# mfkiwl/msckf_stereo_c

Hardware: AMD Instinct MI355X
Metric: stereo frames/sec/node on EuRoC-shape input; ATE RMSE vs CPU ref (higher is better)
Workload: dtype f64

## Files before the change

### msckf_stereo_c_amd/csrc/hip/ekf_linalg.hip

```cpp
#include <mutex>
#include <type_traits>
#include "ekf_device.h"
#include "ekf_cap.h"
#include "chol_block.h"

typedef double v4f64 __attribute__((ext_vector_type(4)));

#define QR_BIAS_LIMIT 1e-6
__device__ __forceinline__ bool ekf_direct_wanted(const EkfStreamDev &S) { return ekf_mode_direct(S.qr_mode, S.rows_out[0], S.rows_out[2]); }
__device__ __forceinline__ bool ekf_skip_gram(const EkfStreamDev &S) { return ekf_mode_householder(S.qr_mode) || ekf_direct_wanted(S); }
__device__ __forceinline__ bool ekf_direct(const EkfStreamDev &S) { return (S.rows_out[3] & 4) != 0; }

template <int MODE> struct GemmTraits;
template <> struct GemmTraits<GM_GRAM> { static constexpr bool TA = true,  SYM = true,  KMIN_I = false, KMIN_J = false; };
template <> struct GemmTraits<GM_T>    { static constexpr bool TA = true,  SYM = false, KMIN_I = true,  KMIN_J = false; };
template <> struct GemmTraits<GM_S2>   { static constexpr bool TA = false, SYM = true,  KMIN_I = false, KMIN_J = true;  };
template <> struct GemmTraits<GM_PUPD> { static constexpr bool TA = true,  SYM = true,  KMIN_I = false, KMIN_J = false; };

#define GT 32
#ifndef GK
#define GK 32
#endif
#define GNE (GK / 8)

template <int MODE>
__global__ __launch_bounds__(256) void k_ekf_gemm(const EkfStreamDev *streams) {
    using TR = GemmTraits<MODE>;
    const EkfStreamDev &S = streams[blockIdx.y];
    if (S.n_feat <= 0) return;
    if (MODE != GM_PUPD && (S.route & EKF_ROUTE_SMALL)) return;
    const int d = S.d, ld = S.ld;
    int gram_tile_i = 0, gram_tile_j = 0;
    EkfCapResult cap = {0, 0, 0, 0ULL};
    if (MODE == GM_GRAM) {
        int tg = 1;
        while ((tg + 1) * (tg + 1) <= (int)gridDim.x) ++tg;
        gram_tile_i = (int)blockIdx.x / tg; gram_tile_j = (int)blockIdx.x - gram_tile_i * tg;
        if (gram_tile_j > gram_tile_i || gram_tile_i * GT > S.na_max) return;
        cap = ekf_cap_local(S, blockIdx.x == 0);
        if (ekf_mode_householder(S.qr_mode) || ekf_mode_direct(S.qr_mode, cap.stacked, cap.na)) return;
    }
    const int na = MODE == GM_GRAM ? cap.na : S.rows_out[2];
    const int *__restrict__ act = S.act;
    const double *__restrict__ A; const double *__restrict__ B; double *C;
    int M, N, K;
    double alpha = 1.0, beta = 0.0, diag_add = 0.0;
    if (MODE == GM_GRAM)      { A = S.Hs; B = S.Hs; C = S.S; M = N = na + 1; K = cap.end; }
    const int nk = MODE == GM_GRAM ? 0 : S.rows_out[4];
    const bool direct = MODE != GM_GRAM && MODE != GM_PUPD && ekf_direct(S);
    if (MODE == GM_T)         { A = direct ? S.Hs : S.S;  B = S.P;  C = S.T; M = nk; N = d; K = na; }
    else if (MODE == GM_S2)   { A = S.T;  B = direct ? S.Hs : S.S;  C = S.W; M = N = nk; K = na; diag_add = S.sigma2; }
    else if (MODE == GM_PUPD) { A = S.T;  B = S.T;  C = S.P; M = N = d; K = nk; alpha = -1.0; beta = 1.0; }
    const int tiles_n = (N + GT - 1) / GT, tiles_m = (M + GT - 1) / GT;
    const int tile = blockIdx.x;
    if (MODE == GM_PUPD && tile >= tiles_m * tiles_n) {
        const int c0 = (tile - tiles_m * tiles_n) * GT;
        if (c0 >= d) return;
        const double *Y = S.T;
        __shared__ double s_part[8][GT + 1];
        const int cl = threadIdx.x & 31, ks = threadIdx.x >> 5;
        const int c = c0 + cl;
        double s2 = 0;
        if (c < d)
            for (int k = ks; k < nk; k += 8) s2 += Y[(size_t)k * ld + c] * Y[(size_t)k * ld + d];
        s_part[ks][cl] = s2;
        __syncthreads();
        if (ks == 0 && c < d) {
            double t = 0;
#pragma unroll
            for (int q = 0; q < 8; ++q) t += s_part[q][cl];
            S.delta_x[c] = t;
        }
        return;
    }
    if (MODE != GM_GRAM && tile >= tiles_m * tiles_n) return;
    const int ti = MODE == GM_GRAM ? gram_tile_i : tile / tiles_n, tj = MODE == GM_GRAM ? gram_tile_j : tile - ti * tiles_n;
    if (MODE == GM_GRAM && ti >= tiles_m) return;
    if (TR::SYM && tj > ti) return;
    const int i0 = ti * GT, j0 = tj * GT;
    __shared__ double sA[GK][GT + 1];
    __shared__ double sB[GK][GT + 1];
    const int tid = threadIdx.x, lane = tid & 63, wave = tid >> 6;
    const int wi = (wave >> 1) * 16, wj = (wave & 1) * 16;
    const int lo = tid & 31, hi = tid >> 5;
    int k_begin = 0;
    if (TR::KMIN_I && !direct) k_begin = (i0 / GK) * GK;
    if (TR::KMIN_J && !direct) k_begin = (j0 / GK) * GK;
    const int k_end = K;
    int colA = i0 + lo, colB = j0 + lo;
    if (MODE == GM_GRAM) {
        colA = (i0 + lo < na) ? ekf_act_column(cap.clones, i0 + lo) : d;
        colB = (j0 + lo < na) ? ekf_act_column(cap.clones, j0 + lo) : d;
    }
    const int cloneA = MODE == GM_GRAM ? (colA < d ? (colA - EKF_IMU_DIM) / 6 : -1) : 0;
    const int cloneB = MODE == GM_GRAM ? (colB < d ? (colB - EKF_IMU_DIM) / 6 : -1) : 0;
    const unsigned long long *__restrict__ rowmask = S.rowmask;
    const int *__restrict__ rowidx = S.act + S.ld;
    double ra[GNE], rb[GNE];
    auto fetch = [&](int k0) {
#pragma unroll
        for (int e = 0; e < GNE; ++e) {
            if (MODE == GM_GRAM) {
                const int gk = k0 + hi + 8 * e;
                double v = 0.0, w = 0.0;
                if (gk < K) {
                    const unsigned long long rm = rowmask[gk];
                    const bool onA = cloneA < 0 ? rm != 0ULL : ((rm >> cloneA) & 1ULL) != 0ULL;
                    const bool onB = cloneB < 0 ? rm != 0ULL : ((rm >> cloneB) & 1ULL) != 0ULL;
                    if (onA && i0 + lo < M) v = A[(size_t)gk * ld + colA];
                    if (onB && j0 + lo < N) w = B[(size_t)gk * ld + colB];
                }
                ra[e] = v; rb[e] = w;
                continue;
            }
            const int ii = TR::TA ? lo : hi + 8 * (e / (GK / 32)), kk = TR::TA ? hi + 8 * e : lo + 32 * (e % (GK / 32));
            const int gi = i0 + ii, gk = k0 + kk;
            double v = 0.0;
            if (gi < M && gk < K && !(TR::KMIN_I && !direct && gk < gi)) {
                if (MODE == GM_S2) v = A[(size_t)gi * ld + act[gk]];
                else if (MODE == GM_T && direct) {
                    const int col = act[gk], ri = rowidx[gi];
                    if ((rowmask[ri] >> ((col - EKF_IMU_DIM) / 6)) & 1ULL) v = A[(size_t)ri * ld + col];
                }
                else v = A[(size_t)gk * ld + (MODE == GM_GRAM ? colA : gi)];
            }
            ra[e] = v;
            const int gj = j0 + lo, gkb = k0 + hi + 8 * e;
            double w = 0.0;
            if (gj < N && gkb < K && !(TR::KMIN_J && !direct && gkb < gj)) {
                if (MODE == GM_T) w = B[(size_t)act[gkb] * ld + gj];
                else if (MODE == GM_S2 && direct) {
                    const int col = act[gkb], rj = rowidx[gj];
                    if ((rowmask[rj] >> ((col - EKF_IMU_DIM) / 6)) & 1ULL) w = B[(size_t)rj * ld + col];
                }
                else w = B[(size_t)gkb * ld + (MODE == GM_GRAM ? colB : gj)];
            }
            rb[e] = w;
        }
    };
    v4f64 acc = {0.0, 0.0, 0.0, 0.0};
    if (k_begin < k_end) fetch(k_begin);
    for (int k0 = k_begin; k0 < k_end; k0 += GK) {
        __syncthreads();
#pragma unroll
        for (int e = 0; e < GNE; ++e) {
            if (TR::TA) sA[hi + 8 * e][lo] = ra[e]; else sA[lo + 32 * (e % (GK / 32))][hi + 8 * (e / (GK / 32))] = ra[e];
            sB[hi + 8 * e][lo] = rb[e];
        }
        __syncthreads();
        if (k0 + GK < k_end) fetch(k0 + GK);
#pragma unroll
        for (int s = 0; s < GK / 4; ++s) {
            const int kk = 4 * s + (lane >> 4);
            const double a = sA[kk][wi + (lane & 15)];
            const double b = sB[kk][wj + (lane & 15)];
            acc = __builtin_amdgcn_mfma_f64_16x16x4f64(a, b, acc, 0, 0, 0);
        }
    }
#pragma unroll
    for (int r = 0; r < 4; ++r) {
        const int i = i0 + wi + (lane >> 4) + 4 * r;
        const int j = j0 + wj + (lane & 15);
        if (i >= M || j >= N) continue;
        if (TR::SYM && j > i) continue;
        double v = alpha * acc[r];
        if (MODE == GM_PUPD) v += beta * C[(size_t)i * ld + j];
        if (i == j) v += diag_add;
        C[(size_t)i * ld + j] = v;
        if (TR::SYM && i != j) C[(size_t)j * ld + i] = v;
        if (MODE == GM_PUPD && i == j && i >= 12 && i < 15 && S.pos_var_out) S.pos_var_out[i - 12] = v;
    }
}

template <int Q> __device__ __forceinline__ double qr_lane_sum(double v) {
    auto bfly = [](double x, auto ctrl) {
        const long long b = __double_as_longlong(x);
        const int lo = __builtin_amdgcn_update_dpp(0, (int)b, decltype(ctrl)::value, 0xf, 0xf, true);
        const int hi = __builtin_amdgcn_update_dpp(0, (int)(b >> 32), decltype(ctrl)::value, 0xf, 0xf, true);
        return x + __longlong_as_double(((long long)hi << 32) | (unsigned int)lo);
    };
    v = bfly(v, std::integral_constant<int, 0xB1>());
    v = bfly(v, std::integral_constant<int, 0x4E>());
    if (Q == 8) v = bfly(v, std::integral_constant<int, 0x141>());
    return v;
}
template <int Q, int RL, class ColOf, class RAt>
__device__ __forceinline__ void tsqr_wide(const EkfStreamDev &S, int n1, int K, ColOf colOf, RAt Rat, double *sB) {
    constexpr int BR = Q * RL;
    const int tid = threadIdx.x, nth = blockDim.x, ld = S.ld;
    const int q = tid & (Q - 1), g = tid / Q, ng = nth / Q;
    for (int k0 = 0; k0 < K; k0 += BR) {
        __syncthreads();
        for (int e = tid; e < BR * n1; e += nth) {
            const int r = e / n1, c = e - r * n1, gk = k0 + r;
            double v = 0.0;
            if (gk < K) {
                int col, clone;
                colOf(c, col, clone);
                const unsigned long long rm = S.rowmask[gk];
                const bool on = clone < 0 ? rm != 0ULL : ((rm >> clone) & 1ULL) != 0ULL;
                if (on) v = S.Hs[(size_t)gk * ld + col];
            }
            sB[e] = v;
        }
        __syncthreads();
        double *own = sB + (size_t)q * RL * n1;
        for (int k = 0; k < n1; ++k) {
            double bk[RL];
            double ss = 0.0;
#pragma unroll
            for (int i = 0; i < RL; ++i) { bk[i] = own[i * n1 + k]; ss += bk[i] * bk[i]; }
            ss = qr_lane_sum<Q>(ss);
            const double x0 = Rat(k, k);
            if (ss < 1e-200 || ss < 1e-40 * (x0 * x0)) continue;
            const double nrm = sqrt(x0 * x0 + ss);
            const double alpha = x0 > 0.0 ? -nrm : nrm;
            const double v0 = x0 - alpha;
            const double beta = 2.0 / (v0 * v0 + ss);
            for (int j = k + 1 + g; j < n1; j += ng) {
                double bj[RL];
                double dot = 0.0;
#pragma unroll
                for (int i = 0; i < RL; ++i) { bj[i] = own[i * n1 + j]; dot += bk[i] * bj[i]; }
                const double rkj = Rat(k, j);
                const double t = beta * (qr_lane_sum<Q>(dot) + v0 * rkj);
#pragma unroll
                for (int i = 0; i < RL; ++i) own[i * n1 + j] = bj[i] - t * bk[i];
                if (q == 0) Rat(k, j) = rkj - t * v0;
            }
            __syncthreads();
            if (tid == 0) Rat(k, k) = alpha;
        }
    }
    __syncthreads();
}
template <class ColOf, class RAt>
__device__ __forceinline__ void tsqr_quads(const EkfStreamDev &S, int n1, int K, ColOf colOf, RAt Rat, double *sB, int room) {
    if (room >= 48 * n1) tsqr_wide<4, 12>(S, n1, K, colOf, Rat, sB);
    else if (room >= 32 * n1) tsqr_wide<4, 8>(S, n1, K, colOf, Rat, sB);
    else tsqr_wide<4, 4>(S, n1, K, colOf, Rat, sB);
}

__device__ __forceinline__ int ekf_compress_entry(const EkfStreamDev &S, int *s_w ) {
    const int na = S.rows_out[2], me = S.rows_out[1], d = S.d, ld = S.ld;
    if (na <= 0) { if (threadIdx.x == 0) S.rows_out[3] = 0; return 1; }
    if (ekf_direct_wanted(S)) {
        int *rowidx = S.act + ld;
        const int tid = threadIdx.x, lane = tid & 63, wave = tid >> 6, nw = (int)blockDim.x >> 6;
        int base = 0;
        for (int r0 = 0; r0 < me; r0 += (int)blockDim.x) {
            const int r = r0 + tid;
            const bool on = r < me && S.rowmask[r] != 0ULL;
            const unsigned long long b = __ballot(on);
            if (lane == 0) s_w[wave] = __popcll(b);
            __syncthreads();
            int off = base, tot = 0;
            for (int w = 0; w < nw; ++w) { const int c = s_w[w]; if (w < wave) off += c; tot += c; }
            if (on && off + __popcll(b & ((1ULL << lane) - 1ULL)) < ld) rowidx[off + __popcll(b & ((1ULL << lane) - 1ULL))] = r;
            base += tot;
            __syncthreads();
        }
        __threadfence_block();
        __syncthreads();
        for (int i = tid; i < base; i += (int)blockDim.x) S.T[(size_t)i * ld + d] = S.Hs[(size_t)rowidx[i] * ld + d];
        if (tid == 0) { S.rows_out[3] = 4; S.rows_out[4] = base; }
        return 1;
    }
    return ekf_skip_gram(S) ? 2 : 0;
}
template <class RAt>
__device__ __forceinline__ void ekf_compress_exit(const EkfStreamDev &S, bool gram_done, int diag, RAt Rat, double *sB, int room) {
    const int na = S.rows_out[2], n1 = na + 1, K = S.rows_out[1], d = S.d, ld = S.ld;
    const int tid = threadIdx.x, nth = blockDim.x;
    const bool need = ekf_mode_householder(S.qr_mode) || (S.qr_mode == 0 && (!gram_done || (diag & 2)));
    if (!need) { if (tid == 0) S.rows_out[3] = diag; return; }
    __syncthreads();
    for (int e = tid; e < n1 * n1; e += nth) { const int k = e / n1, j = e - k * n1; if (j >= k) Rat(k, j) = 0.0; }
    const int *act = S.act;
    tsqr_quads(S, n1, K, [=](int c, int &col, int &clone) { col = c < na ? act[c] : d; clone = c < na ? (col - EKF_IMU_DIM) / 6 : -1; }, Rat, sB, room);
    for (int e = tid; e < na * na; e += nth) {
        const int i = e / na, j = e - i * na;
        if (j <= i) S.S[(size_t)i * ld + j] = Rat(j, i);
    }
    for (int k = tid; k < na; k += nth) S.T[(size_t)k * ld + d] = Rat(k, na);
    if (tid == 0) S.rows_out[3] = diag | 1;
}

#define TQ_THREADS 512
__device__ __forceinline__ double tq_rows_sum(double v) {
    {
        const unsigned long long b = (unsigned long long)__double_as_longlong(v);
        const auto lo = __builtin_amdgcn_permlane16_swap((unsigned)b, (unsigned)b, false, false), hi = __builtin_amdgcn_permlane16_swap((unsigned)(b >> 32), (unsigned)(b >> 32), false, false);
        v = __longlong_as_double((long long)(((unsigned long long)hi[0] << 32) | lo[0])) + __longlong_as_double((long long)(((unsigned long long)hi[1] << 32) | lo[1]));
    }
    {
        const unsigned long long b = (unsigned long long)__double_as_longlong(v);
        const auto lo = __builtin_amdgcn_permlane32_swap((unsigned)b, (unsigned)b, false, false), hi = __builtin_amdgcn_permlane32_swap((unsigned)(b >> 32), (unsigned)(b >> 32), false, false);
        v = __longlong_as_double((long long)(((unsigned long long)hi[0] << 32) | lo[0])) + __longlong_as_double((long long)(((unsigned long long)hi[1] << 32) | lo[1]));
    }
    return v;
}
__device__ __forceinline__ double tq_rcp(double x) {
    double r = __builtin_amdgcn_rcp(x);
    r = __builtin_fma(__builtin_fma(-x, r, 1.0), r, r);
    r = __builtin_fma(__builtin_fma(-x, r, 1.0), r, r);
    return r;
}
template <int C, bool FIRST> __device__ __forceinline__ void tq_fmac_bcast(double &acc, double x, double a) {
    if (FIRST) asm("s_nop 4\n\tv_fmac_f64_dpp %0, %1, %2 row_newbcast:%3 row_mask:0xf bank_mask:0xf" : "+v"(acc) : "v"(x), "v"(a), "n"(C));
    else asm("v_fmac_f64_dpp %0, %1, %2 row_newbcast:%3 row_mask:0xf bank_mask:0xf" : "+v"(acc) : "v"(x), "v"(a), "n"(C));
}
template <int RL, int I = 0> struct TqDot {
    static __device__ __forceinline__ void run(double (&p)[4], const double (&vr)[RL / 16], const double (&bc)[RL]) {
        tq_fmac_bcast<I % 16, I == 0>(p[I & 3], vr[I / 16], bc[I]);
        TqDot<RL, I + 1>::run(p, vr, bc);
    }
};
template <int RL> struct TqDot<RL, RL> { static __device__ __forceinline__ void run(double (&)[4], const double (&)[RL / 16], const double (&)[RL]) {} };
template <int RL, int I = 0> struct TqAxpy {
    static __device__ __forceinline__ void run(double (&bc)[RL], const double (&vr)[RL / 16], double ntt) {
        tq_fmac_bcast<I % 16, I == 0>(bc[I], vr[I / 16], ntt);
        TqAxpy<RL, I + 1>::run(bc, vr, ntt);
    }
};
template <int RL> struct TqAxpy<RL, RL> { static __device__ __forceinline__ void run(double (&)[RL], const double (&)[RL / 16], double) {} };
template <int RL>
__device__ __forceinline__ void tq_form_reflector(const double (&bc)[RL], double x0, double *sVs, int *sFlag_s, double *Rkk, int r) {
    double p0 = 0.0, p1 = 0.0, p2 = 0.0, p3 = 0.0;
#pragma unroll
    for (int i = 0; i < RL; i += 4) { p0 = __builtin_fma(bc[i], bc[i], p0); p1 = __builtin_fma(bc[i + 1], bc[i + 1], p1); p2 = __builtin_fma(bc[i + 2], bc[i + 2], p2); p3 = __builtin_fma(bc[i + 3], bc[i + 3], p3); }
    const double ss = tq_rows_sum((p0 + p1) + (p2 + p3));
    const bool skip = ss < 1e-200 || ss < 1e-40 * (x0 * x0);
    if (!skip) {
        const double n2 = __builtin_fma(x0, x0, ss);
        const double nrm = n2 * rsqrt_nr(n2);
        const double alpha = x0 > 0.0 ? -nrm : nrm;
        const double v0 = x0 - alpha;
        const double beta = 2.0 * tq_rcp(__builtin_fma(v0, v0, ss));
#pragma unroll
        for (int i = 0; i < RL; i += 2) *reinterpret_cast<double2 *>(sVs + r * RL + i) = make_double2(bc[i], bc[i + 1]);
        if (r == 0) { sVs[4 * RL] = v0; sVs[4 * RL + 1] = beta; *Rkk = alpha; }
    }
    if (r == 0) *sFlag_s = skip ? 0 : 1;
}
template <int RL, int NC>
__device__ __forceinline__ void tsqr_regs(const EkfStreamDev &S, int na, int K, double *Rg, double *sV, int *sFlag) {
    static_assert(RL % 16 == 0, "a DPP row holds the reflector's entries of its rows, 16 per register");
    constexpr int BR = 4 * RL, NW = TQ_THREADS / 64, SLAB = 16 * NW, VS = BR + 2, VR = RL / 16;
    const int n1 = na + 1, d = S.d, ld = S.ld;
    const int tid = threadIdx.x, lane = tid & 63, r = lane >> 4, c = lane & 15;
    const int wave = __builtin_amdgcn_readfirstlane(tid >> 6);
    int col[NC], clone[NC];
    bool has[NC];
#pragma unroll
    for (int t = 0; t < NC; ++t) {
        const int j = 16 * wave + c + SLAB * t;
        has[t] = j < n1;
        col[t] = j < na ? S.act[j] : d;
        clone[t] = j < na ? (col[t] - EKF_IMU_DIM) / 6 : -1;
    }
    for (int e = tid; e < n1 * n1; e += TQ_THREADS) { const int k = e / n1, j = e - k * n1; if (j >= k) Rg[(size_t)k * ld + j] = 0.0; }
    __syncthreads();
    for (int k0 = 0; k0 < K; k0 += BR) {
        double b[NC][RL];
#pragma unroll
        for (int i = 0; i < RL; ++i) {
            const int gk = k0 + r * RL + i;
            const unsigned long long rm = gk < K ? S.rowmask[gk] : 0ULL;
#pragma unroll
            for (int t = 0; t < NC; ++t) {
                const bool on = has[t] && (clone[t] < 0 ? rm != 0ULL : ((rm >> clone[t]) & 1ULL) != 0ULL);
                b[t][i] = on ? S.Hs[(size_t)gk * ld + col[t]] : 0.0;
            }
        }
        double ra[NC], rb[NC], rc[NC];
#pragma unroll
        for (int t = 0; t < NC; ++t) {
            const int j = 16 * wave + c + SLAB * t;
            ra[t] = has[t] ? Rg[j] : 0.0;
            rb[t] = has[t] && n1 > 1 ? Rg[(size_t)ld + j] : 0.0;
        }
        if (wave == 0 && c == 0) tq_form_reflector<RL>(b[0], ra[0], sV, sFlag, Rg, r);
        __syncthreads();
        for (int k = 0; k < n1; ++k) {
            const int s = k & 1;
            const double *vs = sV + s * VS;
            double vr[VR];
#pragma unroll
            for (int m = 0; m < VR; ++m) vr[m] = vs[r * RL + 16 * m + c];
            const double v0 = vs[BR], beta = vs[BR + 1];
            const bool live = __builtin_amdgcn_readfirstlane(sFlag[s]) != 0;
#pragma unroll
            for (int t = 0; t < NC; ++t) { const int j = 16 * wave + c + SLAB * t; rc[t] = (has[t] && k + 2 < n1) ? Rg[(size_t)(k + 2) * ld + j] : 0.0; }
            auto apply = [&](double (&bc)[RL], double rkj, int j, bool on) {
                double p[4] = {0.0, 0.0, 0.0, 0.0};
                TqDot<RL>::run(p, vr, bc);
                const double dot = tq_rows_sum((p[0] + p[1]) + (p[2] + p[3]));
                const double tt = on ? beta * __builtin_fma(v0, rkj, dot) : 0.0;
                TqAxpy<RL>::run(bc, vr, -tt);
                if (on && r == 0) Rg[(size_t)k * ld + j] = __builtin_fma(-tt, v0, rkj);
            };
            const int k1 = k + 1;
            const int w1 = (k1 & (SLAB - 1)) >> 4, c1 = k1 & 15, t1 = k1 / SLAB;
            const bool own_wave = k1 < n1 && wave == w1;
#pragma unroll
            for (int t = 0; t < NC; ++t) {
                if (own_wave && t1 == t) {
                    const int j = 16 * wave + c + SLAB * t;
                    if (live) apply(b[t], ra[t], j, has[t] && j > k);
                    if (c == c1) tq_form_reflector<RL>(b[t], rb[t], sV + (s ^ 1) * VS, sFlag + (s ^ 1), Rg + (size_t)k1 * ld + k1, r);
                }
            }
            if (live) {
#pragma unroll
                for (int t = 0; t < NC; ++t) {
                    const int j0 = 16 * wave + SLAB * t;
                    if (!(own_wave && t1 == t) && j0 + 15 > k && j0 < n1) apply(b[t], ra[t], j0 + c, has[t] && j0 + c > k);
                }
            }
#pragma unroll
            for (int t = 0; t < NC; ++t) { ra[t] = rb[t]; rb[t] = rc[t]; }
            __syncthreads();
        }
    }
}
template <int RL, int NC, class Load>
__device__ __forceinline__ void tsqr_wave(int n1, int n_blocks, int first, int stride, Load load, double *R, int ldr, double *sVw, int *sFlagw) {
    constexpr int BR = 4 * RL, VR = RL / 16;
    const int lane = threadIdx.x & 63, r = lane >> 4, c = lane & 15;
    for (int blk = first; blk < n_blocks; blk += stride) {
        double b[NC][RL];
#pragma unroll
        for (int i = 0; i < RL; ++i) {
#pragma unroll
            for (int t = 0; t < NC; ++t) b[t][i] = load(blk, r * RL + i, c + 16 * t);
        }
        for (int k = 0; k < n1; ++k) {
            const int tk = k >> 4, ck = k & 15;
#pragma unroll
            for (int t = 0; t < NC; ++t)
                if (tk == t && c == ck) tq_form_reflector<RL>(b[t], R[k * ldr + k], sVw, sFlagw, R + k * ldr + k, r);
            __builtin_amdgcn_wave_barrier();
            double vr[VR];
#pragma unroll
            for (int m = 0; m < VR; ++m) vr[m] = sVw[r * RL + 16 * m + c];
            const double v0 = sVw[BR], beta = sVw[BR + 1];
            const bool live = __builtin_amdgcn_readfirstlane(*sFlagw) != 0;
            if (live) {
#pragma unroll
                for (int t = 0; t < NC; ++t) {
                    if (16 * t + 15 > k && 16 * t < n1) {
                        const int j = c + 16 * t;
                        const bool on = j < n1 && j > k;
                        const double rkj = on ? R[k * ldr + j] : 0.0;
                        double p[4] = {0.0, 0.0, 0.0, 0.0};
                        TqDot<RL>::run(p, vr, b[t]);
                        const double dot = tq_rows_sum((p[0] + p[1]) + (p[2] + p[3]));
                        const double tt = on ? beta * __builtin_fma(v0, rkj, dot) : 0.0;
                        TqAxpy<RL>::run(b[t], vr, -tt);
                        if (on && r == 0) R[k * ldr + j] = __builtin_fma(-tt, v0, rkj);
                    }
                }
            }
            __builtin_amdgcn_wave_barrier();
        }
    }
}
template <int RL, int NC, int WPE>
__global__ __launch_bounds__(TQ_THREADS, WPE) void k_ekf_tsqr(const EkfStreamDev *streams, int do_cap) {
    const EkfStreamDev &S = streams[blockIdx.y];
    if (S.n_feat <= 0 || (S.route & EKF_ROUTE_SMALL)) return;
    if (!ekf_mode_householder(S.qr_mode)) return;
    if (do_cap) { (void)ekf_cap_local<TQ_THREADS>(S, true); __syncthreads(); }
    __shared__ int s_w[TQ_THREADS / 64];
    __shared__ __attribute__((aligned(16))) double sV[2 * (4 * RL + 2)];
    __shared__ int sFlag[2];
    if (ekf_compress_entry(S, s_w) != 2) return;
    const int na = S.rows_out[2], K = S.rows_out[1], d = S.d, ld = S.ld;
    const int tid = threadIdx.x;
    if (na + 1 > (TQ_THREADS / 4) * NC) { if (tid == 0) S.rows_out[3] = 0x80; return; }
    double *Rg = S.W;
    tsqr_regs<RL, NC>(S, na, K, Rg, sV, sFlag);
    for (int e = tid; e < na * na; e += TQ_THREADS) {
        const int i = e / na, j = e - i * na;
        if (j <= i) S.S[(size_t)i * ld + j] = Rg[(size_t)j * ld + i];
    }
    for (int k = tid; k < na; k += TQ_THREADS) S.T[(size_t)k * ld + d] = Rg[(size_t)k * ld + na];
    if (tid == 0) S.rows_out[3] = 1;
}

#define CHOLG_THREADS 512
__global__ __launch_bounds__(CHOLG_THREADS) void k_ekf_chol(const EkfStreamDev *streams, int which, int pan_rs) {
    const EkfStreamDev &S = streams[blockIdx.y];
    if (S.n_feat <= 0 || (S.route & EKF_ROUTE_SMALL)) return;
    int entry = 0;
    __shared__ int s_w[CHOLG_THREADS / 64];
    if (which == 0) {
        if (ekf_mode_householder(S.qr_mode)) return;
        entry = ekf_compress_entry(S, s_w);
        if (entry == 1) return;
    }
    const int n = which == 0 ? S.rows_out[2] : S.rows_out[4];
    const int nt = n + (which == 0 ? 1 : 0);
    const int lda = S.ld;
    double *A = which == 0 ? S.S : S.W;
    extern __shared__ double s_dyn[];
    double *sPanT = s_dyn;
    __shared__ double s_tol, s_mx[CHOLG_THREADS / 64];
    __shared__ int s_diag;
    __shared__ CholBlockShared s_cb;
    const int tid = threadIdx.x;
    if (tid == 0) s_diag = 0;
    for (int e = tid; e < LNB * pan_rs; e += CHOLG_THREADS) sPanT[e] = 0.0;
    if (which == 0) {
        double mx = 0;
        for (int i = tid; i < n; i += CHOLG_THREADS) mx = fmax(mx, A[(size_t)i * lda + i]);
        for (int off = 32; off > 0; off >>= 1) mx = fmax(mx, __shfl_xor(mx, off));
        if ((tid & 63) == 0) s_mx[tid >> 6] = mx;
        __syncthreads();
        if (tid == 0) { double m = 0; for (int i = 0; i < CHOLG_THREADS / 64; ++i) m = fmax(m, s_mx[i]); s_tol = m * (double)S.d * 1e-14; }
        __syncthreads();
        const double lam = s_tol;
        for (int i = tid; i < n; i += CHOLG_THREADS) A[(size_t)i * lda + i] += lam;
    }
    __syncthreads();
    chol_blocked_lds<CHOLG_THREADS / 64>(A, [lda](int i, int j) { return i * lda + j; }, n, nt, 0.0, sPanT, pan_rs, s_cb);
    if (which == 0) {
        int tiny = 0;
        for (int i = tid; i < n; i += CHOLG_THREADS) { const double l = A[(size_t)i * lda + i]; tiny += (l * l < 100.0 * s_tol) ? 1 : 0; }
        for (int o = 32; o > 0; o >>= 1) tiny += __shfl_xor(tiny, o);
        __shared__ int s_tiny[CHOLG_THREADS / 64];
        if ((tid & 63) == 0) s_tiny[tid >> 6] = tiny;
        __syncthreads();
        double pm = 0;
        for (int i = tid; i < n; i += CHOLG_THREADS) pm = fmax(pm, S.P[(size_t)S.act[i] * lda + S.act[i]]);
        for (int o = 32; o > 0; o >>= 1) pm = fmax(pm, __shfl_xor(pm, o));
        __syncthreads();
        if ((tid & 63) == 0) s_mx[tid >> 6] = pm;
        __syncthreads();
        if (tid == 0) {
            int t = 0; for (int i = 0; i < CHOLG_THREADS / 64; ++i) t += s_tiny[i];
            double p = 0; for (int i = 0; i < CHOLG_THREADS / 64; ++i) p = fmax(p, s_mx[i]);
            s_diag = (t << 8) | ((s_tol * p > QR_BIAS_LIMIT * S.sigma2) ? 2 : 0);
        }
        for (int k = tid; k < n; k += CHOLG_THREADS) S.T[(size_t)k * lda + S.d] = A[(size_t)n * lda + k];
        __syncthreads();
        double *Rg = S.W;
        ekf_compress_exit(S, true, s_diag, [=](int k, int j) -> double & { return Rg[(size_t)k * lda + j]; }, sPanT, LNB * pan_rs);
    }
}

#define CHOL_LDS_MAX_ROWS 181
#define CHOL_THREADS 512
#define CHOL_WAVES (CHOL_THREADS / 64)
#define CHOL_PAN_RS 192

__device__ __forceinline__ int pk(int i, int j) { return i * (i + 1) / 2 + j; }

__global__ __launch_bounds__(CHOL_THREADS) void k_ekf_chol_lds(const EkfStreamDev *streams, int which, int lds_doubles) {
    const EkfStreamDev &S = streams[blockIdx.y];
    if (S.n_feat <= 0 || (S.route & EKF_ROUTE_SMALL)) return;
    int entry = 0;
    __shared__ int s_w[CHOL_WAVES];
    if (which == 0) {
        if (ekf_mode_householder(S.qr_mode)) return;
        entry = ekf_compress_entry(S, s_w);
        if (entry == 1) return;
    }
    double *A = which == 0 ? S.S : S.W;
    const int off = 0, lda = S.ld;
    const int n = which == 0 ? S.rows_out[2] : S.rows_out[4];
    const int nt = n + (which == 0 ? 1 : 0);
    const bool semidef = which == 0;
    extern __shared__ double s_dyn[];
    double *sM = s_dyn;
    double *sPanT = s_dyn + nt * (nt + 1) / 2;
    __shared__ double s_tol, s_mx[CHOL_WAVES];
    __shared__ int s_diag;
    __shared__ CholBlockShared s_cb;
    const int tid = threadIdx.x, lane = tid & 63, wave = tid >> 6;
    if (tid == 0) s_diag = 0;
    auto Rl = [=](int k, int j) -> double & { return sM[k * nt - k * (k - 1) / 2 + (j - k)]; };
    const int room = lds_doubles - nt * (nt + 1) / 2;
    for (int i0 = wave * 8; i0 < nt; i0 += CHOL_WAVES * 8) {
        double v[8][3];
#pragma unroll
        for (int u = 0; u < 8; ++u) {
            const int i = i0 + u;
            const double *src = A + (size_t)(off + i) * lda + off;
#pragma unroll
            for (int k = 0; k < 3; ++k) { const int j = lane + 64 * k; v[u][k] = (i < nt && j <= i) ? src[j] : 0.0; }
        }
#pragma unroll
        for (int u = 0; u < 8; ++u) {
            const int i = i0 + u;
            if (i >= nt) continue;
            double *dst = sM + pk(i, 0);
#pragma unroll
            for (int k = 0; k < 3; ++k) { const int j = lane + 64 * k; if (j <= i) dst[j] = v[u][k]; }
        }
    }
    for (int e = tid; e < LNB * CHOL_PAN_RS; e += CHOL_THREADS) sPanT[e] = 0.0;
    __syncthreads();
    if (semidef) {
        double mx = 0;
        for (int i = tid; i < n; i += CHOL_THREADS) mx = fmax(mx, sM[pk(i, i)]);
        for (int o = 32; o > 0; o >>= 1) mx = fmax(mx, __shfl_xor(mx, o));
        if (lane == 0) s_mx[wave] = mx;
        __syncthreads();
        if (tid == 0) { double m = 0; for (int i = 0; i < CHOL_WAVES; ++i) m = fmax(m, s_mx[i]); s_tol = m * (double)S.d * 1e-14; }
        __syncthreads();
        const double lam = s_tol;
        for (int i = tid; i < n; i += CHOL_THREADS) sM[pk(i, i)] += lam;
        __syncthreads();
    }
    const double tol = 0.0;
    chol_blocked_lds<CHOL_WAVES>(sM, [](int i, int j) { return pk(i, j); }, n, nt, tol, sPanT, CHOL_PAN_RS, s_cb);
    if (which == 0) {
        int tiny = 0;
        for (int i = tid; i < n; i += CHOL_THREADS) { const double l = sM[pk(i, i)]; tiny += (l * l < 100.0 * s_tol) ? 1 : 0; }
        for (int o = 32; o > 0; o >>= 1) tiny += __shfl_xor(tiny, o);
        __shared__ int s_tiny[CHOL_WAVES];
        if (lane == 0) s_tiny[wave] = tiny;
        __syncthreads();
        double pm = 0;
        for (int i = tid; i < n; i += CHOL_THREADS) pm = fmax(pm, S.P[(size_t)S.act[i] * lda + S.act[i]]);
        for (int o = 32; o > 0; o >>= 1) pm = fmax(pm, __shfl_xor(pm, o));
        __syncthreads();
        if (lane == 0) s_mx[wave] = pm;
        __syncthreads();
        if (tid == 0) {
            int t = 0; for (int i = 0; i < CHOL_WAVES; ++i) t += s_tiny[i];
            double p = 0; for (int i = 0; i < CHOL_WAVES; ++i) p = fmax(p, s_mx[i]);
            s_diag = (t << 8) | ((s_tol * p > QR_BIAS_LIMIT * S.sigma2) ? 2 : 0);
        }
    }
    for (int i = wave; i < nt; i += CHOL_WAVES) {
        double *dst = A + (size_t)(off + i) * lda + off;
        const double *src = sM + pk(i, 0);
#pragma unroll
        for (int k = 0; k < 3; ++k) { const int j = lane + 64 * k; if (j <= i && j < n) dst[j] = src[j]; }
    }
    if (which == 0) {
        for (int k = tid; k < n; k += CHOL_THREADS) S.T[(size_t)k * lda + S.d] = sM[pk(n, k)];
        __syncthreads();
        ekf_compress_exit(S, true, s_diag, Rl, sPanT, room);
    }
}

#define QR_MAX_N1 (6 * 64 + 1)
#define TS_COLS 32
#define TS_RB 16
__global__ __launch_bounds__(256) void k_ekf_trsm(const EkfStreamDev *streams) {
    const EkfStreamDev &S = streams[blockIdx.y];
    if (S.n_feat <= 0 || (S.route & EKF_ROUTE_SMALL)) return;
    const int n = S.rows_out[4], ld = S.ld, ncols = S.d + 1;
    const int c0 = blockIdx.x * TS_COLS;
    if (c0 >= ncols) return;
    const double *L = S.W;
    double *B = S.T;
    extern __shared__ double s_dyn[];
    double *sL = s_dyn;
    double *sY = s_dyn + (size_t)TS_RB * (n + 1);
    const int tid = threadIdx.x, c = tid & 31, r8 = tid >> 5;
    for (int e = tid; e < n * TS_COLS; e += 256) {
        const int i = e >> 5, cc = e & 31;
        sY[e] = (c0 + cc < ncols) ? B[(size_t)i * ld + c0 + cc] : 0.0;
    }
    constexpr int LPF = 14;
    const int lrow = tid >> 4, lr = tid & 15;
    double lpf[LPF];
    auto fetch_L = [&](int ib) {
        const int nb = min(TS_RB, n - ib), wcols = ib + nb;
#pragma unroll
        for (int q = 0; q < LPF; ++q) {
            const int p = lr + 16 * q;
            lpf[q] = (lrow < nb && p < wcols) ? L[(size_t)(ib + lrow) * ld + p] : 0.0;
        }
    };
    const bool l_fits = n + TS_RB <= 16 * LPF;
    if (l_fits) fetch_L(0);
    for (int ib = 0; ib < n; ib += TS_RB) {
        const int nb = min(TS_RB, n - ib);
        __syncthreads();
        if (l_fits) {
#pragma unroll
            for (int q = 0; q < LPF; ++q) {
                const int p = lr + 16 * q;
                if (lrow < nb && p < ib + nb) sL[(size_t)lrow * (n + 1) + p] = lpf[q];
            }
            if (ib + TS_RB < n) fetch_L(ib + TS_RB);
        } else {
            for (int e = tid; e < nb * (ib + nb); e += 256) {
                const int i = e / (ib + nb), p = e - i * (ib + nb);
                sL[(size_t)i * (n + 1) + p] = L[(size_t)(ib + i) * ld + p];
            }
        }
        __syncthreads();
        double acc0 = 0.0, acc1 = 0.0;
        {
            const double *l0 = sL + (size_t)r8 * (n + 1), *l1 = sL + (size_t)(r8 + 8) * (n + 1);
            for (int p = 0; p < ib; ++p) {
                const double y = sY[p * TS_COLS + c];
                acc0 += l0[p] * y;
                acc1 += l1[p] * y;
            }
        }
        if (r8 < nb) sY[(ib + r8) * TS_COLS + c] -= acc0;
        if (r8 + 8 < nb) sY[(ib + r8 + 8) * TS_COLS + c] -= acc1;
        __syncthreads();
        if (tid < TS_COLS) {
            double x[TS_RB];
#pragma unroll
            for (int j = 0; j < TS_RB; ++j) {
                x[j] = 0.0;
                if (j < nb) {
                    double s2 = sY[(ib + j) * TS_COLS + tid];
                    const double *lj = sL + (size_t)j * (n + 1) + ib;
#pragma unroll
                    for (int cc = 0; cc < j; ++cc) s2 -= lj[cc] * x[cc];
                    x[j] = (lj[j] != 0.0) ? s2 / lj[j] : 0.0;
                    sY[(ib + j) * TS_COLS + tid] = x[j];
                }
            }
        }
    }
    __syncthreads();
    for (int e = tid; e < n * TS_COLS; e += 256) {
        const int i = e >> 5, cc = e & 31;
        if (c0 + cc < ncols) B[(size_t)i * ld + c0 + cc] = sY[e];
    }
}

#define SU_CH 128
__global__ __launch_bounds__(256) void k_ekf_small_update(const EkfStreamDev *streams) {
    const EkfStreamDev &S = streams[blockIdx.y];
    if (S.n_feat <= 0 || !(S.route & EKF_ROUTE_SMALL)) return;
    const EkfCapResult cap = ekf_cap_local(S, true);
    const int d = S.d, ld = S.ld, na = cap.na, n1 = na + 1, K = cap.end;
    const int tid = threadIdx.x;
    if (na <= 0 || na > SU_MAX_NA) {
        for (int c = tid; c < d; c += 256) S.delta_x[c] = 0.0;
        return;
    }
    extern __shared__ double s_dyn[];
    double *sT = s_dyn;
    double *sG = sT + (size_t)na * (d + 1);
    double *sS = sG + n1 * n1;
    double *sC = sS + na * na;
    __shared__ int s_col[SU_MAX_NA + 1], s_clone[SU_MAX_NA + 1];
    __shared__ double s_lam;
    if (tid < n1) {
        const int col = tid < na ? ekf_act_column(cap.clones, tid) : d;
        s_col[tid] = col;
        s_clone[tid] = tid < na ? (col - EKF_IMU_DIM) / 6 : -1;
    }
    __syncthreads();
    const bool hh_only = ekf_mode_householder(S.qr_mode);
    if (tid == 0) s_lam = 0.0;
    if (!hh_only) {
    const int np = n1 * (n1 + 1) / 2;
    const int groups = np <= 128 ? 256 / np : 1;
    int pi[2], pj[2], pg[2];
    double acc[2] = {0.0, 0.0};
    for (int q = 0; q < 2; ++q) {
        int p = tid + 256 * q, grp = 0;
        if (groups > 1) { grp = q == 0 ? tid / np : groups; p = tid - grp * np; }
        pg[q] = (groups > 1) ? (grp < groups ? grp : -1) : (p < np ? 0 : -1);
        if (pg[q] < 0) p = 0;
        int i = 0;
        while ((i + 1) * (i + 2) / 2 <= p) ++i;
        pi[q] = i; pj[q] = p - i * (i + 1) / 2;
    }
    for (int k0 = 0; k0 < K; k0 += SU_CH) {
        __syncthreads();
        for (int e = tid; e < SU_CH * n1; e += 256) {
            const int r = e / n1, c = e - r * n1, gk = k0 + r;
            double v = 0.0;
            if (gk < K) {
                const unsigned long long rm = S.rowmask[gk];
                const bool on = s_clone[c] < 0 ? rm != 0ULL : ((rm >> s_clone[c]) & 1ULL) != 0ULL;
                if (on) v = S.Hs[(size_t)gk * ld + s_col[c]];
            }
            sC[e] = v;
        }
        __syncthreads();
        for (int q = 0; q < 2; ++q) {
            if (pg[q] < 0) continue;
            double a = acc[q];
            for (int r = pg[q]; r < SU_CH; r += groups) a += sC[r * n1 + pi[q]] * sC[r * n1 + pj[q]];
            acc[q] = a;
        }
    }
    __syncthreads();
    if (groups > 1) {
        if (pg[0] >= 0) sC[pg[0] * np + (pi[0] * (pi[0] + 1) / 2 + pj[0])] = acc[0];
        __syncthreads();
        if (pg[0] == 0) {
            const int p = pi[0] * (pi[0] + 1) / 2 + pj[0];
            double t = 0.0;
            for (int g2 = 0; g2 < groups; ++g2) t += sC[g2 * np + p];
            sG[pi[0] * n1 + pj[0]] = t; sG[pj[0] * n1 + pi[0]] = t;
        }
    } else {
        for (int q = 0; q < 2; ++q)
            if (pg[q] >= 0) { sG[pi[q] * n1 + pj[q]] = acc[q]; sG[pj[q] * n1 + pi[q]] = acc[q]; }
    }
    __syncthreads();
    if (tid == 0) { double mx = 0; for (int i = 0; i < na; ++i) mx = fmax(mx, sG[i * n1 + i]); s_lam = mx * (double)d * 1e-14; }
    __syncthreads();
    if (tid < na) sG[tid * n1 + tid] += s_lam;
    __syncthreads();
    for (int k = 0; k < na; ++k) {
        const double pv = sG[k * n1 + k];
        const double inv = pv > 0.0 ? 1.0 / sqrt(pv) : 0.0;
        __syncthreads();
        if (tid >= k && tid < n1) sG[tid * n1 + k] = (tid == k) ? (pv > 0.0 ? sqrt(pv) : 0.0) : sG[tid * n1 + k] * inv;
        __syncthreads();
        for (int e = tid; e < (n1 - k - 1) * (n1 - k - 1); e += 256) {
            const int i = k + 1 + e / (n1 - k - 1), j = k + 1 + e % (n1 - k - 1);
            if (j <= i) sG[i * n1 + j] -= sG[i * n1 + k] * sG[j * n1 + k];
        }
        __syncthreads();
    }
    }
    {
        __shared__ int s_tiny, s_bias;
        if (tid == 0 && hh_only) { s_tiny = 0; s_bias = 0; }
        if (tid == 0 && !hh_only) {
            int t = 0;
            double pm = 0;
            for (int i = 0; i < na; ++i) {
                const double l = sG[i * n1 + i];
                t += (l * l < 100.0 * s_lam) ? 1 : 0;
                pm = fmax(pm, S.P[(size_t)s_col[i] * ld + s_col[i]]);
            }
            s_tiny = t;
            s_bias = (s_lam * pm > QR_BIAS_LIMIT * S.sigma2) ? 1 : 0;
        }
        __syncthreads();
        const int tiny = s_tiny;
        const bool need_qr = ekf_mode_householder(S.qr_mode) || (S.qr_mode == 0 && (cap.stacked <= na || s_bias));
        if (need_qr) {
            for (int e = tid; e < n1 * n1; e += 256) sG[e] = 0.0;
            __syncthreads();
            static_assert(SU_CH == 128 && SU_MAX_NA + 1 <= 32, "tsqr_wave<32, 2>: 128-row blocks, two 16-column slabs");
            {
                const int wv = __builtin_amdgcn_readfirstlane(tid >> 6);
                double *sRw = sC;
                double *sVq = (double *)(((uintptr_t)(sC + 3 * n1 * n1) + 15) & ~(uintptr_t)15);
                int *sFq = (int *)(sVq + 4 * 130);
                for (int e = tid; e < 3 * n1 * n1; e += 256) sRw[e] = 0.0;
                __syncthreads();
                const unsigned long long *rowmask = S.rowmask;
                const double *Hs = S.Hs;
                auto loadH = [&](int blk, int row, int col) -> double {
                    const int gk = blk * 128 + row;
                    if (gk >= K || col >= n1) return 0.0;
                    const unsigned long long rm = rowmask[gk];
                    const int cl = s_clone[col];
                    const bool on = cl < 0 ? rm != 0ULL : ((rm >> cl) & 1ULL) != 0ULL;
                    return on ? Hs[(size_t)gk * ld + s_col[col]] : 0.0;
                };
                double *Rmine = wv == 0 ? sG : sRw + (wv - 1) * n1 * n1;
                tsqr_wave<32, 2>(n1, (K + 127) / 128, wv, 4, loadH, Rmine, n1, sVq + wv * 130, sFq + wv);
                __syncthreads();
                if (wv == 0) {
                    auto loadR = [&](int, int row, int col) -> double {
                        if (row >= 3 * n1 || col >= n1) return 0.0;
                        const int w2 = row / n1, rr = row - w2 * n1;
                        return col >= rr ? sRw[(w2 * n1 + rr) * n1 + col] : 0.0;
                    };
                    tsqr_wave<32, 2>(n1, 1, 0, 1, loadR, sG, n1, sVq, sFq);
                }
                __syncthreads();
            }
            for (int e = tid; e < n1 * n1; e += 256) { const int i = e / n1, j = e - i * n1; if (j < i) sG[e] = sG[j * n1 + i]; }
            __syncthreads();
        }
        if (tid == 0) S.rows_out[3] = (tiny << 8) | (s_bias ? 2 : 0) | (need_qr ? 1 : 0);
    }
    const double *P = S.P;
    for (int c = tid; c < d; c += 256) {
        double pc[SU_MAX_NA];
#pragma unroll
        for (int k = 0; k < SU_MAX_NA; ++k) pc[k] = k < na ? P[(size_t)s_col[k] * ld + c] : 0.0;
#pragma unroll
        for (int i = 0; i < SU_MAX_NA; ++i) {
            if (i < na) {
                double t = 0.0;
#pragma unroll
                for (int k = i; k < SU_MAX_NA; ++k) if (k < na) t += sG[k * n1 + i] * pc[k];
                sT[i * (d + 1) + c] = t;
            }
        }
    }
    if (tid < na) sT[tid * (d + 1) + d] = sG[na * n1 + tid];
    __syncthreads();
    for (int e = tid; e < na * na; e += 256) {
        const int i = e / na, j = e - i * na;
        if (j > i) continue;
        double t = 0.0;
        for (int k = j; k < na; ++k) t += sT[i * (d + 1) + s_col[k]] * sG[k * n1 + j];
        if (i == j) t += S.sigma2;
        sS[i * na + j] = t; sS[j * na + i] = t;
    }
    __syncthreads();
    for (int k = 0; k < na; ++k) {
        const double pv = sS[k * na + k];
        const double inv = pv > 0.0 ? 1.0 / sqrt(pv) : 0.0;
        __syncthreads();
        if (tid >= k && tid < na) sS[tid * na + k] = (tid == k) ? (pv > 0.0 ? sqrt(pv) : 0.0) : sS[tid * na + k] * inv;
        __syncthreads();
        for (int e = tid; e < (na - k - 1) * (na - k - 1); e += 256) {
            const int i = k + 1 + e / (na - k - 1), j = k + 1 + e % (na - k - 1);
            if (j <= i) sS[i * na + j] -= sS[i * na + k] * sS[j * na + k];
        }
        __syncthreads();
    }
    for (int c = tid; c <= d; c += 256) {
        double y[SU_MAX_NA];
#pragma unroll
        for (int i = 0; i < SU_MAX_NA; ++i) {
            y[i] = 0.0;
            if (i >= na) continue;
            double t = sT[i * (d + 1) + c];
#pragma unroll
            for (int k = 0; k < i; ++k) t -= sS[i * na + k] * y[k];
            const double l = sS[i * na + i];
            y[i] = l != 0.0 ? t / l : 0.0;
            sT[i * (d + 1) + c] = y[i];
        }
    }
    __syncthreads();
    for (int e = tid; e < na * (d + 1); e += 256) {
        const int k = e / (d + 1), c = e - k * (d + 1);
        S.T[(size_t)k * ld + c] = sT[e];
    }
}

extern "C" {
void ekf_launch_gemm(const EkfStreamDev *d, int n, int mode, int max_mn, hipStream_t st) {
    const int t = (max_mn + GT - 1) / GT;
    const dim3 grid(t * t + (mode == GM_PUPD ? t : 0), n);
    switch (mode) {
        case GM_GRAM: hipLaunchKernelGGL(k_ekf_gemm<GM_GRAM>, grid, dim3(256), 0, st, d); break;
        case GM_T:    hipLaunchKernelGGL(k_ekf_gemm<GM_T>, grid, dim3(256), 0, st, d); break;
        case GM_S2:   hipLaunchKernelGGL(k_ekf_gemm<GM_S2>, grid, dim3(256), 0, st, d); break;
        default:      hipLaunchKernelGGL(k_ekf_gemm<GM_PUPD>, grid, dim3(256), 0, st, d); break;
    }
}
void ekf_launch_tsqr(const EkfStreamDev *d, int n, int max_d, int do_cap, hipStream_t st) {
    const int n1 = max_d - EKF_IMU_DIM + 1;
    if (n1 <= 2 * (TQ_THREADS / 4)) hipLaunchKernelGGL((k_ekf_tsqr<32, 2, 2>), dim3(1, n), dim3(TQ_THREADS), 0, st, d, do_cap);
    else hipLaunchKernelGGL((k_ekf_tsqr<16, 4, 2>), dim3(1, n), dim3(TQ_THREADS), 0, st, d, do_cap);
}
void ekf_launch_chol(const EkfStreamDev *d, int n, int which, int max_d, hipStream_t st) {
    const int nt = max_d - EKF_IMU_DIM + 1;
    if (nt <= CHOL_LDS_MAX_ROWS) {
        static std::once_flag attr_once;
    std::call_once(attr_once, []() { (void)hipFuncSetAttribute(reinterpret_cast<const void *>(k_ekf_chol_lds), hipFuncAttributeMaxDynamicSharedMemorySize,
                                      (int)(((size_t)CHOL_LDS_MAX_ROWS * (CHOL_LDS_MAX_ROWS + 1) / 2 + (size_t)CHOL_PAN_RS * LNB) * sizeof(double))); });
        const size_t lds = ((size_t)nt * (nt + 1) / 2 + (size_t)CHOL_PAN_RS * LNB) * sizeof(double);
        hipLaunchKernelGGL(k_ekf_chol_lds, dim3(1, n), dim3(CHOL_THREADS), lds, st, d, which, (int)(lds / sizeof(double)));
        return;
    }
    const int pan_rs = (nt + 15) / 16 * 16;
    hipLaunchKernelGGL(k_ekf_chol, dim3(1, n), dim3(CHOLG_THREADS), (size_t)LNB * pan_rs * sizeof(double), st, d, which, pan_rs);
}
void ekf_launch_small_update(const EkfStreamDev *d, int n, int max_d, hipStream_t st) {
    const size_t lds = ((size_t)SU_MAX_NA * (max_d + 1) + (SU_MAX_NA + 1) * (SU_MAX_NA + 1) + SU_MAX_NA * SU_MAX_NA + SU_CH * (SU_MAX_NA + 1)) * sizeof(double);
    static std::once_flag attr_once;
    std::call_once(attr_once, []() {
        hipFuncAttributes fa;
        size_t stat = 4096;
        if (hipFuncGetAttributes(&fa, reinterpret_cast<const void *>(k_ekf_small_update)) == hipSuccess) stat = fa.sharedSizeBytes;
        if (hipFuncSetAttribute(reinterpret_cast<const void *>(k_ekf_small_update), hipFuncAttributeMaxDynamicSharedMemorySize, (int)(160 * 1024 - stat)) != hipSuccess) (void)hipGetLastError();
    });
    hipLaunchKernelGGL(k_ekf_small_update, dim3(1, n), dim3(256), lds, st, d);
}
void ekf_launch_trsm(const EkfStreamDev *d, int n, int max_d, hipStream_t st) {
    const int strips = (max_d + 1 + TS_COLS - 1) / TS_COLS;
    const int max_n = max_d > EKF_IMU_DIM ? max_d - EKF_IMU_DIM : 1;
    const size_t lds = (size_t)(TS_RB * (max_n + 1) + (size_t)max_n * TS_COLS) * sizeof(double);
    static std::once_flag attr_once;
    std::call_once(attr_once, []() { (void)hipFuncSetAttribute(reinterpret_cast<const void *>(k_ekf_trsm), hipFuncAttributeMaxDynamicSharedMemorySize, 160 * 1024); });
    hipLaunchKernelGGL(k_ekf_trsm, dim3(strips, n), dim3(256), lds, st, d);
}
}
```

Measured before the change: 98660.

## Panel-block the register TSQR to cut block barriers and batch H loads

Restructures the register-resident Householder TSQR so that reflectors are formed in panels of PW columns by the owning wave, using wave-level barriers. Other waves then apply the whole panel between block-wide barriers, instead of synchronising after every column. It also restructures the H-row loads in both TSQR paths: row masks and H entries are fetched in bulk and masked afterwards, so loads can be issued ahead. The trade-off is larger shared staging for PW reflectors and a longer serial panel-factor phase on one wave, with possible load imbalance.

```diff
diff --git a/msckf_stereo_c_amd/csrc/hip/ekf_linalg.hip b/msckf_stereo_c_amd/csrc/hip/ekf_linalg.hip
--- a/msckf_stereo_c_amd/csrc/hip/ekf_linalg.hip
+++ b/msckf_stereo_c_amd/csrc/hip/ekf_linalg.hip
@@ -287,6 +287,9 @@
 }
 
 #define TQ_THREADS 512
+#ifndef TQ_PANEL
+#define TQ_PANEL 16
+#endif
 __device__ __forceinline__ double tq_rows_sum(double v) {
     {
         const unsigned long long b = (unsigned long long)__double_as_longlong(v);
@@ -343,83 +346,137 @@
     }
     if (r == 0) *sFlag_s = skip ? 0 : 1;
 }
-template <int RL, int NC>
-__device__ __forceinline__ void tsqr_regs(const EkfStreamDev &S, int na, int K, double *Rg, double *sV, int *sFlag) {
+__device__ __forceinline__ int tq_lane() {
+    int l = (int)__builtin_amdgcn_mbcnt_hi(~0u, __builtin_amdgcn_mbcnt_lo(~0u, 0u));
+    asm volatile("" : "+v"(l));
+    return l;
+}
+template <int RL, int NC, int PW>
+__device__ __forceinline__ void tsqr_regs(const EkfStreamDev &S, int na, int K, double *Rg, double *sP, int *sPF) {
     static_assert(RL % 16 == 0, "a DPP row holds the reflector's entries of its rows, 16 per register");
+    static_assert(PW == 16 || PW == 8, "a panel is a slab of a wavefront or half of one");
     constexpr int BR = 4 * RL, NW = TQ_THREADS / 64, SLAB = 16 * NW, VS = BR + 2, VR = RL / 16;
     const int n1 = na + 1, d = S.d, ld = S.ld;
-    const int tid = threadIdx.x, lane = tid & 63, r = lane >> 4, c = lane & 15;
-    const int wave = __builtin_amdgcn_readfirstlane(tid >> 6);
-    int col[NC], clone[NC];
-    bool has[NC];
-#pragma unroll
-    for (int t = 0; t < NC; ++t) {
-        const int j = 16 * wave + c + SLAB * t;
-        has[t] = j < n1;
-        col[t] = j < na ? S.act[j] : d;
-        clone[t] = j < na ? (col[t] - EKF_IMU_DIM) / 6 : -1;
-    }
-    for (int e = tid; e < n1 * n1; e += TQ_THREADS) { const int k = e / n1, j = e - k * n1; if (j >= k) Rg[(size_t)k * ld + j] = 0.0; }
+    const int wave = __builtin_amdgcn_readfirstlane((int)threadIdx.x >> 6);
+    const int NP = (n1 + PW - 1) / PW;
+    for (int e = threadIdx.x; e < n1 * n1; e += TQ_THREADS) { const int k = e / n1, j = e - k * n1; if (j >= k) Rg[(size_t)k * ld + j] = 0.0; }
     __syncthreads();
     for (int k0 = 0; k0 < K; k0 += BR) {
         double b[NC][RL];
-#pragma unroll
-        for (int i = 0; i < RL; ++i) {
-            const int gk = k0 + r * RL + i;
-            const unsigned long long rm = gk < K ? S.rowmask[gk] : 0ULL;
+        {
+            const int ln = tq_lane(), g0 = k0 + (ln >> 4) * RL, j0 = 16 * wave + (ln & 15);
+            unsigned long long rm[RL];
+            int col[NC], clone[NC];
+            bool has[NC];
 #pragma unroll
             for (int t = 0; t < NC; ++t) {
-                const bool on = has[t] && (clone[t] < 0 ? rm != 0ULL : ((rm >> clone[t]) & 1ULL) != 0ULL);
-                b[t][i] = on ? S.Hs[(size_t)gk * ld + col[t]] : 0.0;
-            }
-        }
-        double ra[NC], rb[NC], rc[NC];
-#pragma unroll
-        for (int t = 0; t < NC; ++t) {
-            const int j = 16 * wave + c + SLAB * t;
-            ra[t] = has[t] ? Rg[j] : 0.0;
-            rb[t] = has[t] && n1 > 1 ? Rg[(size_t)ld + j] : 0.0;
-        }
-        if (wave == 0 && c == 0) tq_form_reflector<RL>(b[0], ra[0], sV, sFlag, Rg, r);
-        __syncthreads();
-        for (int k = 0; k < n1; ++k) {
-            const int s = k & 1;
-            const double *vs = sV + s * VS;
-            double vr[VR];
-#pragma unroll
-            for (int m = 0; m < VR; ++m) vr[m] = vs[r * RL + 16 * m + c];
-            const double v0 = vs[BR], beta = vs[BR + 1];
-            const bool live = __builtin_amdgcn_readfirstlane(sFlag[s]) != 0;
-#pragma unroll
-            for (int t = 0; t < NC; ++t) { const int j = 16 * wave + c + SLAB * t; rc[t] = (has[t] && k + 2 < n1) ? Rg[(size_t)(k + 2) * ld + j] : 0.0; }
-            auto apply = [&](double (&bc)[RL], double rkj, int j, bool on) {
-                double p[4] = {0.0, 0.0, 0.0, 0.0};
-                TqDot<RL>::run(p, vr, bc);
-                const double dot = tq_rows_sum((p[0] + p[1]) + (p[2] + p[3]));
-                const double tt = on ? beta * __builtin_fma(v0, rkj, dot) : 0.0;
-                TqAxpy<RL>::run(bc, vr, -tt);
-                if (on && r == 0) Rg[(size_t)k * ld + j] = __builtin_fma(-tt, v0, rkj);
-            };
-            const int k1 = k + 1;
-            const int w1 = (k1 & (SLAB - 1)) >> 4, c1 = k1 & 15, t1 = k1 / SLAB;
-            const bool own_wave = k1 < n1 && wave == w1;
+                const int j = j0 + SLAB * t;
+                has[t] = j < n1;
+                col[t] = j < na ? S.act[j] : d;
+                clone[t] = j < na ? (col[t] - EKF_IMU_DIM) / 6 : -1;
+            }
+#pragma unroll
+            for (int i = 0; i < RL; ++i) { const int gk = g0 + i; rm[i] = gk < K ? S.rowmask[gk] : 0ULL; }
+#pragma unroll
+            for (int i = 0; i < RL; ++i) {
+                const int gk = min(g0 + i, K - 1);
+#pragma unroll
+                for (int t = 0; t < NC; ++t) b[t][i] = S.Hs[(unsigned)(gk * ld + col[t])];
+            }
+#pragma unroll
+            for (int i = 0; i < RL; ++i) {
+#pragma unroll
+                for (int t = 0; t < NC; ++t) {
+                    const bool on = has[t] && (clone[t] < 0 ? rm[i] != 0ULL : ((rm[i] >> clone[t]) & 1ULL) != 0ULL);
+                    b[t][i] = on ? b[t][i] : 0.0;
+                }
+            }
+        }
+        auto apply = [&](double (&bc)[RL], const double (&vr)[VR], double v0, double beta, double rkj, int k, int j, bool on, bool top) {
+            double p[4] = {0.0, 0.0, 0.0, 0.0};
+            TqDot<RL>::run(p, vr, bc);
+            const double dot = tq_rows_sum((p[0] + p[1]) + (p[2] + p[3]));
+            const double tt = on ? beta * __builtin_fma(v0, rkj, dot) : 0.0;
+            TqAxpy<RL>::run(bc, vr, -tt);
+            if (on && top) Rg[(unsigned)(k * ld + j)] = __builtin_fma(-tt, v0, rkj);
+        };
+        auto apply_panel = [&](int p, double (&bc)[RL], int q) {
+            const int ln = tq_lane(), lo = (ln >> 4) * RL + (ln & 15), j = 16 * q + (ln & 15);
+            const bool on = j < n1, top = ln < 16;
+            const int kp = p * PW, np = min(PW, n1 - kp);
+            const double *pv = sP + (p & 1) * (PW * VS);
+            const int *pf = sPF + (p & 1) * PW;
+            double ra = on ? Rg[(unsigned)(kp * ld + j)] : 0.0;
+            double rb = on && np > 1 ? Rg[(unsigned)((kp + 1) * ld + j)] : 0.0;
+            double vr[VR], v0, beta;
+            int fl;
+#pragma unroll
+            for (int m = 0; m < VR; ++m) vr[m] = pv[lo + 16 * m];
+            v0 = pv[BR]; beta = pv[BR + 1]; fl = pf[0];
+            for (int kk = 0; kk < np; ++kk) {
+                const double rc = on && kk + 2 < np ? Rg[(unsigned)((kp + kk + 2) * ld + j)] : 0.0;
+                const double *pn = pv + min(kk + 1, np - 1) * VS;
+                double vn[VR];
+#pragma unroll
+                for (int m = 0; m < VR; ++m) vn[m] = pn[lo + 16 * m];
+                const double v0n = pn[BR], betan = pn[BR + 1];
+                const int fn = pf[min(kk + 1, np - 1)];
+                if (__builtin_amdgcn_readfirstlane(fl) != 0) apply(bc, vr, v0, beta, ra, kp + kk, j, on, top);
+#pragma unroll
+                for (int m = 0; m < VR; ++m) vr[m] = vn[m];
+                v0 = v0n; beta = betan; fl = fn;
+                ra = rb; rb = rc;
+            }
+        };
+        auto factor = [&](int p) {
+            const int kp = p * PW, np = min(PW, n1 - kp), tp = kp / SLAB, c0 = kp & 15;
+            double *pv = sP + (p & 1) * (PW * VS);
+            int *pf = sPF + (p & 1) * PW;
 #pragma unroll
             for (int t = 0; t < NC; ++t) {
-                if (own_wave && t1 == t) {
-                    const int j = 16 * wave + c + SLAB * t;
-                    if (live) apply(b[t], ra[t], j, has[t] && j > k);
-                    if (c == c1) tq_form_reflector<RL>(b[t], rb[t], sV + (s ^ 1) * VS, sFlag + (s ^ 1), Rg + (size_t)k1 * ld + k1, r);
+                if (t == tp) {
+                    const int ln = tq_lane(), r = ln >> 4, c = ln & 15, lo = r * RL + c, j = 16 * wave + c + SLAB * t;
+                    const bool has = j < n1;
+                    double ra = has ? Rg[(unsigned)(kp * ld + j)] : 0.0;
+                    double rb = has && np > 1 ? Rg[(unsigned)((kp + 1) * ld + j)] : 0.0;
+                    for (int cc = 0; cc < np; ++cc) {
+                        const int k = kp + cc;
+                        const double rc = has && cc + 2 < np ? Rg[(unsigned)((k + 2) * ld + j)] : 0.0;
+                        double *ps = pv + cc * VS;
+                        if (j == k) tq_form_reflector<RL>(b[t], ra, ps, pf + cc, Rg + (unsigned)(k * ld + k), r);
+                        __builtin_amdgcn_wave_barrier();
+                        if (c0 + cc < 15 && k + 1 < n1) {
+                            double vr[VR];
+#pragma unroll
+                            for (int m = 0; m < VR; ++m) vr[m] = ps[lo + 16 * m];
+                            const double v0 = ps[BR], beta = ps[BR + 1];
+                            if (__builtin_amdgcn_readfirstlane(pf[cc]) != 0) apply(b[t], vr, v0, beta, ra, k, j, has && j > k, r == 0);
+                        }
+                        __builtin_amdgcn_wave_barrier();
+                        ra = rb; rb = rc;
+                    }
                 }
             }
-            if (live) {
-#pragma unroll
-                for (int t = 0; t < NC; ++t) {
-                    const int j0 = 16 * wave + SLAB * t;
-                    if (!(own_wave && t1 == t) && j0 + 15 > k && j0 < n1) apply(b[t], ra[t], j0 + c, has[t] && j0 + c > k);
+        };
+        if (wave == 0) factor(0);
+        __syncthreads();
+        for (int p = 0; p < NP; ++p) {
+            const int qp = (p * PW) >> 4, q1 = ((p + 1) * PW) >> 4;
+            const bool own_next = p + 1 < NP && wave == (q1 & (NW - 1));
+            const int t1 = q1 / NW;
+            if (own_next) {
+                if (q1 > qp) {
+#pragma unroll
+                    for (int t = 0; t < NC; ++t)
+                        if (t == t1) apply_panel(p, b[t], q1);
                 }
-            }
-#pragma unroll
-            for (int t = 0; t < NC; ++t) { ra[t] = rb[t]; rb[t] = rc[t]; }
+                factor(p + 1);
+            }
+#pragma unroll
+            for (int t = 0; t < NC; ++t) {
+                const int q = wave + NW * t;
+                if (!(own_next && t == t1) && q > qp && 16 * q < n1) apply_panel(p, b[t], q);
+            }
             __syncthreads();
         }
     }
@@ -430,11 +487,7 @@
     const int lane = threadIdx.x & 63, r = lane >> 4, c = lane & 15;
     for (int blk = first; blk < n_blocks; blk += stride) {
         double b[NC][RL];
-#pragma unroll
-        for (int i = 0; i < RL; ++i) {
-#pragma unroll
-            for (int t = 0; t < NC; ++t) b[t][i] = load(blk, r * RL + i, c + 16 * t);
-        }
+        load(blk, r * RL, c, b);
         for (int k = 0; k < n1; ++k) {
             const int tk = k >> 4, ck = k & 15;
 #pragma unroll
@@ -466,21 +519,21 @@
         }
     }
 }
-template <int RL, int NC, int WPE>
+template <int RL, int NC, int WPE, int PW = TQ_PANEL>
 __global__ __launch_bounds__(TQ_THREADS, WPE) void k_ekf_tsqr(const EkfStreamDev *streams, int do_cap) {
     const EkfStreamDev &S = streams[blockIdx.y];
     if (S.n_feat <= 0 || (S.route & EKF_ROUTE_SMALL)) return;
     if (!ekf_mode_householder(S.qr_mode)) return;
     if (do_cap) { (void)ekf_cap_local<TQ_THREADS>(S, true); __syncthreads(); }
     __shared__ int s_w[TQ_THREADS / 64];
-    __shared__ __attribute__((aligned(16))) double sV[2 * (4 * RL + 2)];
-    __shared__ int sFlag[2];
+    __shared__ __attribute__((aligned(16))) double sP[2 * PW * (4 * RL + 2)];
+    __shared__ int sPF[2 * PW];
     if (ekf_compress_entry(S, s_w) != 2) return;
     const int na = S.rows_out[2], K = S.rows_out[1], d = S.d, ld = S.ld;
     const int tid = threadIdx.x;
     if (na + 1 > (TQ_THREADS / 4) * NC) { if (tid == 0) S.rows_out[3] = 0x80; return; }
     double *Rg = S.W;
-    tsqr_regs<RL, NC>(S, na, K, Rg, sV, sFlag);
+    tsqr_regs<RL, NC, PW>(S, na, K, Rg, sP, sPF);
     for (int e = tid; e < na * na; e += TQ_THREADS) {
         const int i = e / na, j = e - i * na;
         if (j <= i) S.S[(size_t)i * ld + j] = Rg[(size_t)j * ld + i];
@@ -854,22 +907,43 @@
                 __syncthreads();
                 const unsigned long long *rowmask = S.rowmask;
                 const double *Hs = S.Hs;
-                auto loadH = [&](int blk, int row, int col) -> double {
-                    const int gk = blk * 128 + row;
-                    if (gk >= K || col >= n1) return 0.0;
-                    const unsigned long long rm = rowmask[gk];
-                    const int cl = s_clone[col];
-                    const bool on = cl < 0 ? rm != 0ULL : ((rm >> cl) & 1ULL) != 0ULL;
-                    return on ? Hs[(size_t)gk * ld + s_col[col]] : 0.0;
+                auto loadH = [&](int blk, int row0, int c, double (&bb)[2][32]) {
+                    unsigned long long rm[32];
+                    int colx[2], cl[2];
+                    bool has[2];
+#pragma unroll
+                    for (int t = 0; t < 2; ++t) { const int col = c + 16 * t; has[t] = col < n1; colx[t] = s_col[has[t] ? col : 0]; cl[t] = s_clone[has[t] ? col : 0]; }
+#pragma unroll
+                    for (int i = 0; i < 32; ++i) { const int gk = blk * 128 + row0 + i; rm[i] = gk < K ? rowmask[gk] : 0ULL; }
+#pragma unroll
+                    for (int i = 0; i < 32; ++i) {
+                        const int gk = min(blk * 128 + row0 + i, K - 1);
+#pragma unroll
+                        for (int t = 0; t < 2; ++t) bb[t][i] = Hs[(size_t)gk * ld + colx[t]];
+                    }
+#pragma unroll
+                    for (int i = 0; i < 32; ++i) {
+#pragma unroll
+                        for (int t = 0; t < 2; ++t) {
+                            const bool on = has[t] && (cl[t] < 0 ? rm[i] != 0ULL : ((rm[i] >> cl[t]) & 1ULL) != 0ULL);
+                            bb[t][i] = on ? bb[t][i] : 0.0;
+                        }
+                    }
                 };
                 double *Rmine = wv == 0 ? sG : sRw + (wv - 1) * n1 * n1;
                 tsqr_wave<32, 2>(n1, (K + 127) / 128, wv, 4, loadH, Rmine, n1, sVq + wv * 130, sFq + wv);
                 __syncthreads();
                 if (wv == 0) {
-                    auto loadR = [&](int, int row, int col) -> double {
-                        if (row >= 3 * n1 || col >= n1) return 0.0;
-                        const int w2 = row / n1, rr = row - w2 * n1;
-                        return col >= rr ? sRw[(w2 * n1 + rr) * n1 + col] : 0.0;
+                    auto loadR = [&](int, int row0, int c, double (&bb)[2][32]) {
+#pragma unroll
+                        for (int i = 0; i < 32; ++i) {
+#pragma unroll
+                            for (int t = 0; t < 2; ++t) {
+                                const int row = row0 + i, col = c + 16 * t;
+                                const int w2 = row / n1, rr = row - w2 * n1;
+                                bb[t][i] = (row < 3 * n1 && col < n1 && col >= rr) ? sRw[(w2 * n1 + rr) * n1 + col] : 0.0;
+                            }
+                        }
                     };
                     tsqr_wave<32, 2>(n1, 1, 0, 1, loadR, sG, n1, sVq, sFq);
                 }
```

New measurement: 95780. 0.971x the previous value.
